# KMASAHIRO/AVR

Hardware: AMD Instinct MI355X
Metric: ray-samples/sec/GPU (1024 rays×256 samp×512 freq) + IR render ms/pose (higher is better)
Workload: dtype f32; 1 GPU; c2_meshrir_1024x256x512; mode=pose, rays=1024, samples=256, T=1022, freq_bins=512, distinct_poses=16, parallelism=poses x1 (no data-path collective)

## Files before the change

### avr_amd/csrc/render_bwd.hip

```cpp
#include "common.h"

using namespace avr;

typedef float floatx4 __attribute__((ext_vector_type(4)));

namespace {

constexpr int kBwdThreads = 256;
constexpr int kFc = 32;

__global__ __launch_bounds__(kBwdThreads) void dft_phase_bwd_kernel(
    avr_render_params pp, const float2* __restrict__ gout, const float* __restrict__ pl,
    const float2* __restrict__ phase, const float2* __restrict__ twg, float* __restrict__ gz, int B,
    int S, int T) {
    extern __shared__ float2 tw[];
    __shared__ float Au[16][kFc + 1];
    __shared__ float Av[16][kFc + 1];
    const int F = T / 2 + 1;
    const int b = blockIdx.z;
    const int s0 = blockIdx.y * 16;
    const int wave = threadIdx.x >> 6, lane = threadIdx.x & 63;
    const int t = blockIdx.x * 64 + wave * 16 + (lane & 15);
    const int tm = (t < T) ? t : 0;
    const int kq = lane >> 4;
    const int fo = kq >> 1, comp = kq & 1;
    const int srow = threadIdx.x >> 4, scol = 2 * (threadIdx.x & 15);
    const int ss = min(s0 + srow, S - 1);
    float2 ph_raw[2], g_raw[2];
    auto issue = [&](int fc) {
#pragma unroll
        for (int q = 0; q < 2; ++q) {
            const int f = min(fc + scol + q, F - 1);
            g_raw[q] = gout[(int64_t)b * F + f];
            ph_raw[q] = phase[(int64_t)ss * F + f];
        }
    };
    auto commit = [&](int fc) {
#pragma unroll
        for (int q = 0; q < 2; ++q) {
            const bool ok = (s0 + srow) < S && (fc + scol + q) < F;
            const float2 g = g_raw[q], ph = ph_raw[q];
            Au[srow][scol + q] = ok ? g.x * ph.x + g.y * ph.y : 0.0f;
            Av[srow][scol + q] = ok ? -(g.x * ph.y - g.y * ph.x) : 0.0f;
        }
    };
    issue(0);
    stage_table<kBwdThreads>(tw, twg, T);
    floatx4 acc = {0.0f, 0.0f, 0.0f, 0.0f};
    const int inc = (int)((2LL * tm) % T);
    for (int fc = 0; fc < F; fc += kFc) {
        __syncthreads();
        commit(fc);
        __syncthreads();
        if (fc + kFc < F) issue(fc + kFc);
        int idx = (int)(((int64_t)(fc + fo) * tm) % T);
#pragma unroll 4
        for (int ff = 0; ff < kFc; ff += 2) {
            const int r = lane & 15;
            const float a = comp ? Av[r][ff + fo] : Au[r][ff + fo];
            const float2 c = tw[idx];
            const float bv = comp ? c.y : c.x;
            acc = __builtin_amdgcn_mfma_f32_16x16x4f32(a, bv, acc, 0, 0, 0);
            idx += inc;
            if (idx >= T) idx -= T;
        }
    }
    float g4[4];
    int sh4[4];
#pragma unroll
    for (int reg = 0; reg < 4; ++reg) {
        const int s = min(s0 + 4 * kq + reg, S - 1);
        sh4[reg] = receiver_shift(pp, s);
        g4[reg] = pl[sh4[reg] + min(tm, T - 1)];
    }
    if (t < T) {
#pragma unroll
        for (int reg = 0; reg < 4; ++reg) {
            const int s = s0 + 4 * kq + reg;
            if (s < S) {
                const float v = (t < T - 1 - sh4[reg]) ? acc[reg] * g4[reg] : 0.0f;
                gz[((int64_t)b * S + s) * T + t] = v;
            }
        }
    }
}

constexpr int kMaxRbThreads = 1024;
constexpr int kMaxRbRays = 4096;

template <typename Tin, bool VECTOR, int CPT, int G, int MAXT, bool NTS>
__global__ __launch_bounds__(MAXT) void ray_reduce_bwd_kernel(
    avr_render_params pp, const Tin* __restrict__ sig, const float* __restrict__ gz, const float* __restrict__ w,
    const int32_t* __restrict__ delay, Tin* __restrict__ gsig, float* __restrict__ gw, int B,
    int R, int S, int T, int rays_per_split, int64_t total) {
    constexpr int VEC = VECTOR ? Vec16<Tin>::N : 1;
    extern __shared__ float lds_rb[];
    const int nthreads = blockDim.x, lane = threadIdx.x & 63;
    const int split = blockIdx.x, s0 = blockIdx.y * G, b = blockIdx.z;
    const int gcount = min(G, S - s0);
    const int r0 = split * rays_per_split;
    const int nr = max(0, min(R, r0 + rays_per_split) - r0);
    const int stride_l = G * max(nr, 1);
    float* w_l = lds_rb;
    int* d_l = reinterpret_cast<int*>(lds_rb + stride_l);
    float* dot_l = lds_rb + 2 * stride_l;
    for (int i = threadIdx.x; i < G * nr; i += nthreads) {
        const int g = i / nr, rr = i - g * nr;
        dot_l[i] = 0.0f;
        if (g < gcount) {
            const int64_t idx = ((int64_t)b * R + r0 + rr) * S + s0 + g;
            w_l[i] = w[idx];
            d_l[i] = delay[idx];
        } else {
            w_l[i] = 0.0f;
            d_l[i] = 0x7fffffff;
        }
    }
    const int64_t row0 = (((int64_t)b * R + r0) * S + s0) * (int64_t)T;
    const int L = gcount * T;
    const int phase = (int)(row0 % VEC);
    const int nchunks = (L + phase + VEC - 1) / VEC;
    const int64_t row_stride = (int64_t)S * T;

    float gv[CPT][VEC];
    int tk[CPT][VEC];
    int tm[CPT][VEC];
    int gk[CPT][VEC];
    int tmax[CPT][G];
    int lim[G];
    bool full[CPT];
    const float* gzc = gz + ((int64_t)b * S + s0) * T;
#pragma unroll
    for (int g = 0; g < G; ++g) lim[g] = tail_limit(pp, min(s0 + g, S - 1));
#pragma unroll
    for (int c = 0; c < CPT; ++c) {
        const int j = threadIdx.x + c * nthreads;
        const int ebase = j * VEC - phase;
        full[c] = j < nchunks && ebase >= 0 && ebase + VEC <= L;
#pragma unroll
        for (int g = 0; g < G; ++g) tmax[c][g] = -1;
#pragma unroll
        for (int k = 0; k < VEC; ++k) {
            const int e = ebase + k;
            const bool ok = j < nchunks && e >= 0 && e < L;
            const int g = (G == 1) ? 0 : (ok ? e / T : 0);
            gk[c][k] = g;
            tk[c][k] = ok ? e - g * T : -1;
            gv[c][k] = ok ? gzc[e] : 0.0f;
            int l = lim[0];
#pragma unroll
            for (int q = 1; q < G; ++q)
                if (g == q) l = lim[q];
            tm[c][k] = (tk[c][k] >= 0 && tk[c][k] < l) ? tk[c][k] : -1;
#pragma unroll
            for (int q = 0; q < G; ++q)
                if (g == q) tmax[c][q] = max(tmax[c][q], tm[c][k]);
        }
    }
    __syncthreads();

    auto live = [&](int r, int c) {
        bool any = false;
#pragma unroll
        for (int g = 0; g < G; ++g) any |= tmax[c][g] >= d_l[g * nr + r];
        return any;
    };
    auto load_chunk = [&](int64_t rowbase, int c, bool need, float* x) {
        const int j = threadIdx.x + c * nthreads;
        if constexpr (VECTOR) {
            load16_masked(sig + rowbase, (uint32_t)nchunks * 16u,
                          need ? (uint32_t)j * 16u : kSkip, x);
        } else {
            const int64_t e0 = rowbase + j;
            x[0] = (need && j < nchunks && e0 < total) ? load_f(sig, e0) : 0.0f;
        }
    };
    auto finish = [&](int r, int64_t rowbase, float (*x)[VEC]) {
        float wg[G], dotg[G];
        int dg[G];
#pragma unroll
        for (int g = 0; g < G; ++g) {
            wg[g] = w_l[g * nr + r];
            dg[g] = d_l[g * nr + r];
            dotg[g] = 0.0f;
        }
#pragma unroll
        for (int c = 0; c < CPT; ++c) {
            float o[VEC];
#pragma unroll
            for (int k = 0; k < VEC; ++k) {
                float ws = wg[0];
                int ds = dg[0];
#pragma unroll
                for (int g = 1; g < G; ++g)
                    if (gk[c][k] == g) {
                        ws = wg[g];
                        ds = dg[g];
                    }
                const float gm = (tm[c][k] >= ds) ? gv[c][k] : 0.0f;
                o[k] = ws * gm;
                const float pd = gm * x[c][k];
#pragma unroll
                for (int g = 0; g < G; ++g)
                    if (gk[c][k] == g) dotg[g] += pd;
            }
            const int j = threadIdx.x + c * nthreads;
            const int64_t e0 = rowbase + (int64_t)j * VEC;
            if (VECTOR && full[c]) {
                if constexpr (VECTOR) {
                    if constexpr (NTS)
                        store16_nt(gsig + e0, o);
                    else
                        store16(gsig + e0, o);
                }
            } else {
#pragma unroll
                for (int k = 0; k < VEC; ++k)
                    if (tk[c][k] >= 0) store_f(gsig, e0 + k, o[k]);
            }
        }
#pragma unroll
        for (int g = 0; g < G; ++g) {
            float v = dotg[g];
#pragma unroll
            for (int off = 32; off > 0; off >>= 1) v += __shfl_xor(v, off, 64);
            if (lane == 0) atomicAdd(&dot_l[g * nr + r], v);
        }
    };

    constexpr int U = 4;
    int r = 0;
    for (; r + U <= nr; r += U) {
        float x[U][CPT][VEC];
        bool need[U][CPT];
#pragma unroll
        for (int u = 0; u < U; ++u)
#pragma unroll
            for (int c = 0; c < CPT; ++c) need[u][c] = live(r + u, c);
#pragma unroll
        for (int u = 0; u < U; ++u) {
            const int64_t bu = row0 + (int64_t)(r + u) * row_stride - phase;
#pragma unroll
            for (int c = 0; c < CPT; ++c) load_chunk(bu, c, need[u][c], x[u][c]);
        }
#pragma unroll
        for (int u = 0; u < U; ++u) finish(r + u, row0 + (int64_t)(r + u) * row_stride - phase, x[u]);
    }
    for (; r < nr; ++r) {
        float xa[CPT][VEC];
        const int64_t ba = row0 + (int64_t)r * row_stride - phase;
#pragma unroll
        for (int c = 0; c < CPT; ++c) load_chunk(ba, c, live(r, c), xa[c]);
        finish(r, ba, xa);
    }
    __syncthreads();
    for (int i = threadIdx.x; i < G * nr; i += nthreads) {
        const int g = i / nr, rr = i - g * nr;
        if (g < gcount) gw[((int64_t)b * R + r0 + rr) * S + s0 + g] = dot_l[i];
    }
}

template <typename Ta>
__global__ void weights_bwd_kernel(avr_render_params p, int B, const Ta* __restrict__ attn,
                                   const float* __restrict__ d_vals,
                                   const float* __restrict__ grad_w, Ta* __restrict__ grad_attn,
                                   int waves_per_block) {
    extern __shared__ float lds[];
    const int R = n_rays(p), S = p.n_samples;
    const int wave = threadIdx.x >> 6, lane = threadIdx.x & 63;
    const int64_t ray = (int64_t)blockIdx.x * waves_per_block + wave;
    const bool active = ray < (int64_t)B * R;
    float* alpha = lds + (int64_t)wave * 4 * S;
    float* gwl = alpha + S;
    float* ex = gwl + S;
    float* dist = ex + S;
    const int64_t base = ray * S;
    if (active) {
        for (int s = lane; s < S; s += 64) {
            const float a = load_f(attn, base + s);
            const float d = d_vals[s];
            const float gap = (s + 1 < S) ? d_vals[s + 1] - d : 1e10f;
            const float e = expf(-a * gap);
            alpha[s] = 1.0f - e;
            ex[s] = e;
            dist[s] = gap;
            gwl[s] = grad_w[base + s];
        }
    }
    __syncthreads();
    if (!active) return;
    const int per = (S + 63) / 64;
    const int s0 = min(S, lane * per), s1 = min(S, s0 + per);
    float run = 1.0f;
    for (int s = s0; s < s1; ++s) run = run * ((1.0f - alpha[s]) + 1e-6f);
    float incl = run;
#pragma unroll
    for (int off = 1; off < 64; off <<= 1) {
        const float v = __shfl_up(incl, off, 64);
        if (lane >= off) incl = incl * v;
    }
    float trans0 = __shfl_up(incl, 1, 64);
    if (lane == 0) trans0 = 1.0f;
    float ca = 0.0f, cm = 1.0f;
    for (int s = s1 - 1; s >= s0; --s) {
        const float a_s = gwl[s] * alpha[s];
        const float m_s = (1.0f - alpha[s]) + 1e-6f;
        ca = a_s + m_s * ca;
        cm = m_s * cm;
    }
    float qa = ca, qm = cm;
#pragma unroll
    for (int off = 1; off < 64; off <<= 1) {
        const float na = __shfl_down(qa, off, 64);
        const float nm = __shfl_down(qm, off, 64);
        if (lane + off < 64) {
            qa = qa + qm * na;
            qm = qm * nm;
        }
    }
    float q = __shfl_down(qa, 1, 64);
    if (lane == 63) q = 0.0f;
    for (int s = s1 - 1; s >= s0; --s) {
        const float u_s = q;
        q = gwl[s] * alpha[s] + ((1.0f - alpha[s]) + 1e-6f) * q;
        gwl[s] = gwl[s] - u_s;
    }
    float tr = trans0;
    for (int s = s0; s < s1; ++s) {
        const float galpha = tr * gwl[s];
        const float gatt = (galpha * ex[s]) * dist[s];
        store_f(grad_attn, base + s, gatt);
        tr = tr * ((1.0f - alpha[s]) + 1e-6f);
    }
}

}

extern "C" int avr_dft_phase_bwd(const avr_render_params* p, int32_t B, const float* grad_out,
                                 const float* pl_table, const int32_t* shift, const float* phase,
                                 const float* twiddle, float* gz, void* stream) {
    AVR_REQUIRE(p && B >= 1 && grad_out && pl_table && shift && phase && twiddle && gz,
                "avr_dft_phase_bwd: bad args");
    const int S = p->n_samples, T = p->T;
    AVR_REQUIRE(T >= 2 && T <= 16384, "avr_dft_phase_bwd: T out of range");
    const dim3 grid((T + 63) / 64, (S + 15) / 16, B);
    const size_t lds = (size_t)T * sizeof(float2);
    (void)shift;
    if (lds > 65536)
        (void)hipFuncSetAttribute((const void*)dft_phase_bwd_kernel,
                                  hipFuncAttributeMaxDynamicSharedMemorySize, (int)lds);
    hipLaunchKernelGGL(dft_phase_bwd_kernel, grid, dim3(kBwdThreads), lds, as_stream(stream), *p,
                       reinterpret_cast<const float2*>(grad_out), pl_table,
                       reinterpret_cast<const float2*>(phase),
                       reinterpret_cast<const float2*>(twiddle), gz, (int)B, S, T);
    return check_launch("avr_dft_phase_bwd");
}

namespace {
template <typename Tin, bool VECTOR>
int launch_rb(const avr_render_params* p, int B, const void* sig, const float* gz, const float* w,
              const int32_t* delay, void* gsig, float* gw, hipStream_t st) {
    constexpr int VEC = VECTOR ? Vec16<Tin>::N : 1;
    const int R = n_rays(*p), S = p->n_samples, T = p->T;
    int G = 1;
    const int max_chunks = (VEC == 8) ? 256 : 512;
    while (G < 4 && 2 * G * T <= max_chunks * VEC && 2 * G <= S) G *= 2;
    int max_phase = 0;
    for (int s0 = 0; s0 < S && s0 < VEC * G; s0 += G)
        max_phase = max(max_phase, (int)(((int64_t)s0 * T) % VEC));
    const int nch = (G * T + max_phase + VEC - 1) / VEC;
    int cpt = 1;
    while ((nch + cpt - 1) / cpt > kMaxRbThreads) ++cpt;
    const int threads = max(64, ((nch + cpt - 1) / cpt + 63) / 64 * 64);
    const int groups = (S + G - 1) / G;
    int n = 1;
    const int64_t wps = (int64_t)groups * B * (threads / 64);
    const int64_t waves_target = 262144;
    auto rps_of = [&](int k) { return (R + k - 1) / k; };
    while (n < 256 && (n * wps < waves_target || rps_of(n) * G > kMaxRbRays) && rps_of(2 * n) >= 4) n *= 2;
    const int rps = rps_of(n);
    if (rps * G > kMaxRbRays) return fail(AVR_E_CONFIG, "ray_reduce_bwd: too many rays per split");
    const int64_t total = (int64_t)B * R * S * T;
    const dim3 grid((R + rps - 1) / rps, groups, B);
    const size_t lds = (size_t)3 * G * max(rps, 1) * 4;
    const Tin* x = (const Tin*)sig;
    Tin* gx = (Tin*)gsig;
    const bool nts = true;
#define AVR_RB_L(C, GG, MT, NTS)                                                                   \
    hipLaunchKernelGGL((ray_reduce_bwd_kernel<Tin, VECTOR, C, GG, MT, NTS>), grid, dim3(threads),  \
                       lds, st, *p, x, gz, w, delay, gx, gw, B, R, S, T, rps, total)
#define AVR_RB(C, GG)                                                                              \
    if (cpt == C && G == GG) {                                                                     \
        if (threads <= 512) {                                                                      \
            if (nts)                                                                               \
                AVR_RB_L(C, GG, 512, true);                                                        \
            else                                                                                   \
                AVR_RB_L(C, GG, 512, false);                                                       \
        } else {                                                                                   \
            if (nts)                                                                               \
                AVR_RB_L(C, GG, 1024, true);                                                       \
            else                                                                                   \
                AVR_RB_L(C, GG, 1024, false);                                                      \
        }                                                                                          \
        return check_launch("avr_ray_reduce_bwd");                                                 \
    }
    AVR_RB(1, 1) AVR_RB(1, 2) AVR_RB(1, 4) AVR_RB(2, 1) AVR_RB(2, 2) AVR_RB(2, 4) AVR_RB(3, 1)
    AVR_RB(4, 1)
#undef AVR_RB_L
#undef AVR_RB
    return fail(AVR_E_CONFIG, "ray_reduce_bwd: T too long for this build");
}
}

extern "C" int avr_ray_reduce_bwd(const avr_render_params* p, int32_t B, const void* signal,
                                  int32_t sig_dtype, const float* gz, const float* w,
                                  const int32_t* delay, void* grad_signal, float* grad_w,
                                  void* stream) {
    AVR_REQUIRE(p && B >= 1 && signal && gz && w && delay && grad_signal && grad_w,
                "avr_ray_reduce_bwd: bad args");
    AVR_REQUIRE(p->T >= 2 && p->T <= 16384, "avr_ray_reduce_bwd: T out of range");
    const int64_t st = (int64_t)p->n_samples * p->T;
    const bool aligned = (reinterpret_cast<uintptr_t>(signal) % 16) == 0 &&
                         (reinterpret_cast<uintptr_t>(grad_signal) % 16) == 0;
    hipStream_t s = as_stream(stream);
    if (sig_dtype == AVR_DTYPE_F32) {
        if (aligned && st % 4 == 0)
            return launch_rb<float, true>(p, B, signal, gz, w, delay, grad_signal, grad_w, s);
        return launch_rb<float, false>(p, B, signal, gz, w, delay, grad_signal, grad_w, s);
    }
    if (sig_dtype == AVR_DTYPE_F16) {
        if (aligned && st % 8 == 0)
            return launch_rb<__half, true>(p, B, signal, gz, w, delay, grad_signal, grad_w, s);
        return launch_rb<__half, false>(p, B, signal, gz, w, delay, grad_signal, grad_w, s);
    }
    if (sig_dtype == AVR_DTYPE_BF16) {
        if (aligned && st % 8 == 0)
            return launch_rb<__hip_bfloat16, true>(p, B, signal, gz, w, delay, grad_signal, grad_w, s);
        return launch_rb<__hip_bfloat16, false>(p, B, signal, gz, w, delay, grad_signal, grad_w, s);
    }
    return fail(AVR_E_ARG, "avr_ray_reduce_bwd: unknown signal dtype");
}

extern "C" int avr_weights_bwd(const avr_render_params* p, int32_t B, const void* attn,
                               int32_t attn_dtype, const float* d_vals, const float* grad_w,
                               void* grad_attn, void* stream) {
    AVR_REQUIRE(p && B >= 1 && attn && d_vals && grad_w && grad_attn, "avr_weights_bwd: bad args");
    const int S = p->n_samples;
    AVR_REQUIRE(S >= 1 && S <= 8192, "avr_weights_bwd: n_samples out of range");
    const int wpb = (S <= 1024) ? 4 : 1;
    const int64_t rays = (int64_t)B * n_rays(*p);
    const dim3 grid((unsigned)((rays + wpb - 1) / wpb));
    const size_t lds = (size_t)wpb * 4 * S * sizeof(float);
    if (lds > 65536) {
        if (attn_dtype == AVR_DTYPE_F32)
            (void)hipFuncSetAttribute((const void*)weights_bwd_kernel<float>,
                                hipFuncAttributeMaxDynamicSharedMemorySize, (int)lds);
        else if (attn_dtype == AVR_DTYPE_F16)
            (void)hipFuncSetAttribute((const void*)weights_bwd_kernel<__half>,
                                hipFuncAttributeMaxDynamicSharedMemorySize, (int)lds);
        else
            (void)hipFuncSetAttribute((const void*)weights_bwd_kernel<__hip_bfloat16>,
                                hipFuncAttributeMaxDynamicSharedMemorySize, (int)lds);
    }
    if (attn_dtype == AVR_DTYPE_F32)
        hipLaunchKernelGGL(weights_bwd_kernel<float>, grid, dim3(64 * wpb), lds, as_stream(stream),
                           *p, (int)B, (const float*)attn, d_vals, grad_w, (float*)grad_attn, wpb);
    else if (attn_dtype == AVR_DTYPE_F16)
        hipLaunchKernelGGL(weights_bwd_kernel<__half>, grid, dim3(64 * wpb), lds,
                           as_stream(stream), *p, (int)B, (const __half*)attn, d_vals, grad_w,
                           (__half*)grad_attn, wpb);
    else if (attn_dtype == AVR_DTYPE_BF16)
        hipLaunchKernelGGL(weights_bwd_kernel<__hip_bfloat16>, grid, dim3(64 * wpb), lds,
                           as_stream(stream), *p, (int)B, (const __hip_bfloat16*)attn, d_vals, grad_w,
                           (__hip_bfloat16*)grad_attn, wpb);
    else
        return fail(AVR_E_ARG, "avr_weights_bwd: unknown attn dtype");
    return check_launch("avr_weights_bwd");
}
```

### avr_amd/csrc/render_fwd.hip

```cpp
#include "common.h"

#include <cstdlib>

using namespace avr;

typedef float floatx16 __attribute__((ext_vector_type(16)));

namespace {

constexpr double kTwoPi = 6.283185307179586476925286766559;

__global__ void tables_kernel(avr_render_params p, float* __restrict__ d_vals,
                              float* __restrict__ frac, int32_t* __restrict__ shift,
                              float* __restrict__ pl, float2* __restrict__ phase,
                              float2* __restrict__ tw) {
    const int S = p.n_samples, T = p.T, F = T / 2 + 1;
    const int64_t gid = (int64_t)blockIdx.x * blockDim.x + threadIdx.x;
    const int64_t stride = (int64_t)gridDim.x * blockDim.x;
    for (int64_t i = gid; i < S; i += stride) {
        const float d = linspace_at(0.0f, 1.0f, S, (int)i) * p.depth_scale + p.depth_offset;
        const float fr = (p.fs * d) / p.speed;
        d_vals[i] = d;
        frac[i] = fr;
        shift[i] = (int32_t)rintf(fr);
// ... 239 lines not shown
        for (int s = lane; s < S; s += 64) w_out[base + s] = alpha[s];
}

constexpr int kMaxReduceThreads = 1024;
constexpr int kMaxGroupRays = 4096;

template <typename Tin, bool VECTOR, int CPT, int kUnroll, int G, int MAXT>
__global__ __launch_bounds__(MAXT) void ray_reduce_fwd_kernel(
    avr_render_params pp, const Tin* __restrict__ sig, const float* __restrict__ w,
    const int32_t* __restrict__ delay, float* __restrict__ part, int B, int R, int S, int T,
    int rays_per_split, int64_t total) {
    constexpr int VEC = VECTOR ? Vec16<Tin>::N : 1;
    extern __shared__ float lds_wd[];
    const int nthreads = blockDim.x;
    const int split = blockIdx.x, s0 = blockIdx.y * G, b = blockIdx.z;
    const int gcount = min(G, S - s0);
    const int r0 = split * rays_per_split;
    const int nr = max(0, min(R, r0 + rays_per_split) - r0);
    float* w_l = lds_wd;
    int* d_l = reinterpret_cast<int*>(lds_wd + G * max(nr, 1));
    for (int i = threadIdx.x; i < G * nr; i += nthreads) {
        const int g = i / nr, rr = i - g * nr;
        if (g < gcount) {
            const int64_t idx = ((int64_t)b * R + r0 + rr) * S + s0 + g;
            w_l[i] = w[idx];
            d_l[i] = delay[idx];
        } else {
            w_l[i] = 0.0f;
            d_l[i] = 0x7fffffff;
        }
    }
    __syncthreads();
    const int64_t row0 = (((int64_t)b * R + r0) * S + s0) * (int64_t)T;
    const int L = gcount * T;
    const int phase = (int)(row0 % VEC);
    const int nchunks = (L + phase + VEC - 1) / VEC;
    const int64_t row_stride = (int64_t)S * T;

    float acc[CPT][VEC];
    int tk[CPT][VEC];
    int tm[CPT][VEC];
    int gk[CPT][VEC];
    int tmax[CPT][G];
    int lim[G];
#pragma unroll
    for (int g = 0; g < G; ++g) lim[g] = tail_limit(pp, min(s0 + g, S - 1));
#pragma unroll
    for (int c = 0; c < CPT; ++c) {
#pragma unroll
        for (int g = 0; g < G; ++g) tmax[c][g] = -1;
#pragma unroll
        for (int k = 0; k < VEC; ++k) {
            acc[c][k] = 0.0f;
            const int e = (threadIdx.x + c * nthreads) * VEC + k - phase;
            const bool ok = e >= 0 && e < L;
            const int g = (G == 1) ? 0 : (ok ? e / T : 0);
            gk[c][k] = g;
            tk[c][k] = ok ? e - g * T : -1;
            int l = lim[0];
#pragma unroll
            for (int q = 1; q < G; ++q)
                if (g == q) l = lim[q];
            tm[c][k] = (tk[c][k] >= 0 && tk[c][k] < l) ? tk[c][k] : -1;
#pragma unroll
            for (int q = 0; q < G; ++q)
                if (g == q) tmax[c][q] = max(tmax[c][q], tm[c][k]);
        }
    }

    auto live = [&](int r, int c) {
        bool any = false;
#pragma unroll
        for (int g = 0; g < G; ++g) any |= tmax[c][g] >= d_l[g * nr + r];
        return any;
    };
    auto load_chunk = [&](int64_t rowbase, int c, bool need, float* x) {
        const int j = threadIdx.x + c * nthreads;
        if constexpr (VECTOR) {
            load16_masked(sig + rowbase, (uint32_t)nchunks * 16u,
                          need ? (uint32_t)j * 16u : kSkip, x);
        } else {
            const int64_t e0 = rowbase + j;
            x[0] = (need && j < nchunks && e0 < total) ? load_f(sig, e0) : 0.0f;
        }
    };
    auto accumulate = [&](int r, float (*x)[VEC]) {
        float wg[G];
        int dg[G];
#pragma unroll
        for (int g = 0; g < G; ++g) {
            wg[g] = w_l[g * nr + r];
            dg[g] = d_l[g * nr + r];
        }
#pragma unroll
        for (int c = 0; c < CPT; ++c)
#pragma unroll
            for (int k = 0; k < VEC; ++k) {
                float ws = wg[0];
                int ds = dg[0];
#pragma unroll
                for (int g = 1; g < G; ++g)
                    if (gk[c][k] == g) {
                        ws = wg[g];
                        ds = dg[g];
                    }
                const float wm = (tm[c][k] >= ds) ? ws : 0.0f;
                acc[c][k] = fmaf(wm, x[c][k], acc[c][k]);
            }
    };

    int r = 0;
    for (; r + kUnroll <= nr; r += kUnroll) {
        float x[kUnroll][CPT][VEC];
        bool need[kUnroll][CPT];
#pragma unroll
        for (int u = 0; u < kUnroll; ++u)
#pragma unroll
            for (int c = 0; c < CPT; ++c) need[u][c] = live(r + u, c);
#pragma unroll
        for (int u = 0; u < kUnroll; ++u) {
            const int64_t rowbase = row0 + (int64_t)(r + u) * row_stride - phase;
#pragma unroll
            for (int c = 0; c < CPT; ++c) load_chunk(rowbase, c, need[u][c], x[u][c]);
        }
#pragma unroll
        for (int u = 0; u < kUnroll; ++u) accumulate(r + u, x[u]);
    }
    for (; r < nr; ++r) {
        const int64_t rowbase = row0 + (int64_t)r * row_stride - phase;
        float x[CPT][VEC];
#pragma unroll
        for (int c = 0; c < CPT; ++c) load_chunk(rowbase, c, live(r, c), x[c]);
        accumulate(r, x);
    }
#pragma unroll
    for (int c = 0; c < CPT; ++c)
#pragma unroll
        for (int k = 0; k < VEC; ++k) {
            const int t = tk[c][k];
            if (t >= 0) part[(((int64_t)split * B + b) * S + s0 + gk[c][k]) * T + t] = acc[c][k];
        }
}

constexpr int kDftThreads = 256;
constexpr int kKc = 64;

template <int NS>
__global__ __launch_bounds__(kDftThreads) void dft_phase_fwd_kernel(
    avr_render_params pp, const float* __restrict__ part, const float* __restrict__ pl,
    const int32_t* __restrict__ shift, const float2* __restrict__ phase,
    const float2* __restrict__ twg, float2* __restrict__ spart, int B, int S, int T, int KS,
    int kchunk, int xcd_order) {
    extern __shared__ float2 tw[];
    __shared__ float As[32][kKc + 1];
    const int F = T / 2 + 1;
    const int P = ((S + 31) / 32) * KS;
    (void)P;
    const int nfb = (F + 127) / 128, nst = (S + 31) / 32;
    const int per = KS * nfb;
    int stile, q;
    if (xcd_order) {
        const int L = blockIdx.x, xcd = L & 7;
        q = L >> 3;
        stile = (q / per) * 8 + xcd;
        if (stile >= nst) return;
    } else {
        stile = blockIdx.x / per;
        q = blockIdx.x;
    }
    const int ks = (q % per) / nfb, fblk = (q % per) % nfb;
    const int b = blockIdx.z;
    const int wave = threadIdx.x >> 6, lane = threadIdx.x & 63;
    const int fbase = fblk * 128 + wave * 32;
    const int f = fbase + (lane & 31);
    const int fm = (f < F) ? f : 0;
    const int half = lane >> 5;
    const int col = threadIdx.x & 63, row0 = threadIdx.x >> 6;
    int sh[8];
    bool srow[8];
#pragma unroll
    for (int i = 0; i < 8; ++i) {
        const int s = stile * 32 + row0 + 4 * i;
        srow[i] = s < S;
        sh[i] = receiver_shift(pp, min(s, S - 1));
    }
    (void)shift;
    const int64_t slab = (int64_t)B * S * T;
    const int s_first = min(stile * 32 + row0, S - 1);
    const int64_t rowbase0 = ((int64_t)b * S + s_first) * T;
    const int64_t max_row_off = ((int64_t)b * S + (S - 1)) * T;

    const int k0 = ks * kchunk;
    const int k1 = min(T, k0 + kchunk);
    floatx16 acc_re, acc_im;
#pragma unroll
    for (int i = 0; i < 16; ++i) {
        acc_re[i] = 0.0f;
        acc_im[i] = 0.0f;
    }
    const int inc = (int)((2LL * fm) % T);
    float raw[NS][8], g[8];
    auto issue = [&](int kc) {
        const int tc = min(kc + col, T - 1);
#pragma unroll
        for (int k = 0; k < NS; ++k)
#pragma unroll
            for (int i = 0; i < 8; ++i) {
                const int64_t ro = min(rowbase0 + (int64_t)(4 * i) * T, max_row_off);
                raw[k][i] = part[k * slab + ro + tc];
            }
#pragma unroll
        for (int i = 0; i < 8; ++i) g[i] = pl[sh[i] + tc];
    };
    auto commit = [&](int kc) {
        const int t = kc + col;
#pragma unroll
        for (int i = 0; i < 8; ++i) {
            float sum = raw[0][i];
#pragma unroll
            for (int k = 1; k < NS; ++k) sum += raw[k][i];
            const bool ok = srow[i] && t < k1 && t < T - 1 - sh[i];
            As[row0 + 4 * i][col] = ok ? sum * g[i] : 0.0f;
        }
    };
    if (k0 < k1) issue(k0);
    stage_table<kDftThreads>(tw, twg, T);
    for (int kc = k0; kc < k1; kc += kKc) {
        __syncthreads();
        commit(kc);
        __syncthreads();
        if (kc + kKc < k1) issue(kc + kKc);
        int idx = (int)(((int64_t)(kc + half) * fm) % T);
#pragma unroll 8
        for (int kk = 0; kk < kKc; kk += 2) {
            const float a = As[lane & 31][kk + half];
            float2 c = tw[idx];
            asm volatile("" : "+v"(c.x), "+v"(c.y));
            acc_re = __builtin_amdgcn_mfma_f32_32x32x2f32(a, c.x, acc_re, 0, 0, 0);
            acc_im = __builtin_amdgcn_mfma_f32_32x32x2f32(a, c.y, acc_im, 0, 0, 0);
            idx += inc;
            if (idx >= T) idx -= T;
        }
    }
    float re = 0.0f, im = 0.0f;
    {
        float2 ph[16];
#pragma unroll
        for (int reg = 0; reg < 16; ++reg) {
            const int s = stile * 32 + (reg & 3) + 8 * (reg >> 2) + 4 * half;
            ph[reg] = phase[(int64_t)min(s, S - 1) * F + fm];
        }
#pragma unroll
        for (int reg = 0; reg < 16; ++reg) asm volatile("" ::"v"(ph[reg].x), "v"(ph[reg].y));
#pragma unroll
        for (int reg = 0; reg < 16; ++reg) {
            const int s = stile * 32 + (reg & 3) + 8 * (reg >> 2) + 4 * half;
            if (s < S) {
                const float zr = acc_re[reg], zi = acc_im[reg];
                re += zr * ph[reg].x - zi * ph[reg].y;
                im += zr * ph[reg].y + zi * ph[reg].x;
            }
        }
    }
    re += __shfl_xor(re, 32, 64);
    im += __shfl_xor(im, 32, 64);
    if (half == 0 && f < F) {
        spart[((int64_t)b * P + stile * KS + ks) * F + f] = make_float2(re, im);
    }
}

__global__ __launch_bounds__(256) void spectrum_finalize_kernel(int B, int P, int F,
                                                                const float2* __restrict__ spart,
                                                                float2* __restrict__ out) {
    __shared__ float2 red[16][17];
    const int b = blockIdx.y;
    const int g = threadIdx.x >> 4, j = threadIdx.x & 15;
    const int f = blockIdx.x * 16 + j;
    const int fc = min(f, F - 1);
    const float2* src = spart + (int64_t)b * P * F + fc;
    float ax = 0.f, ay = 0.f;
    for (int q0 = 0; q0 < P; q0 += 64) {
        float2 v[4];
#pragma unroll
        for (int u = 0; u < 4; ++u) v[u] = src[(int64_t)min(q0 + g + 16 * u, P - 1) * F];
#pragma unroll
        for (int u = 0; u < 4; ++u)
            if (q0 + g + 16 * u < P) {
                ax += v[u].x;
                ay += v[u].y;
            }
    }
    red[g][j] = make_float2(ax, ay);
    __syncthreads();
    if (g == 0 && f < F) {
        float2 r = red[0][j];
        for (int k = 1; k < 16; ++k) {
            r.x += red[k][j].x;
            r.y += red[k][j].y;
        }
        out[(int64_t)b * F + f] = r;
    }
}

__global__ __launch_bounds__(256) void irfft_kernel(int F, int B1, const float2* __restrict__ spec,
                                                    const float2* __restrict__ spec2,
                                                    const float2* __restrict__ twg,
                                                    float* __restrict__ ir, float* __restrict__ ir2) {
    extern __shared__ float2 lds[];
    __shared__ float red[8][33];
    const int n = 2 * (F - 1);
    float2* X = lds;
    float2* tw = lds + F;
    int b = blockIdx.y;
    if (b >= B1) {
        b -= B1;
        spec = spec2;
        ir = ir2;
    }
    stage_table<256>(X, spec + (int64_t)b * F, F);
    stage_table<256>(tw, twg, n);
    __syncthreads();
    const int tl = threadIdx.x & 31, slice = threadIdx.x >> 5;
    const int t = blockIdx.x * 32 + tl;
    const int tm = (t < n) ? t : 0;
    float acc[4] = {0.f, 0.f, 0.f, 0.f};
    int idx[4];
#pragma unroll
    for (int c = 0; c < 4; ++c) idx[c] = (int)(((int64_t)(1 + slice + 8 * c) * tm) % n);
    const int step4 = (int)((32LL * tm) % n);
    int k = 1 + slice;
    for (; k + 24 < F - 1; k += 32) {
#pragma unroll
        for (int c = 0; c < 4; ++c) {
            const float2 w = tw[idx[c]];
            const float2 x = X[k + 8 * c];
            acc[c] += x.x * w.x - x.y * w.y;
            idx[c] += step4;
            if (idx[c] >= n) idx[c] -= n;
        }
    }
    for (; k < F - 1; k += 8) {
        const int id = (int)(((int64_t)k * tm) % n);
        const float2 w = tw[id];
        const float2 x = X[k];
        acc[0] += x.x * w.x - x.y * w.y;
    }
    red[slice][tl] = (acc[0] + acc[1]) + (acc[2] + acc[3]);
    __syncthreads();
    if (slice == 0 && t < n) {
        float s = 0.0f;
#pragma unroll
        for (int q = 0; q < 8; ++q) s += red[q][tl];
        const float nyq = (t & 1) ? -X[F - 1].x : X[F - 1].x;
        const float v = (X[0].x + nyq) + 2.0f * s;
        ir[(int64_t)b * n + t] = v / (float)n;
    }
}

__global__ __launch_bounds__(256) void irfft_bwd_kernel(int F, const float* __restrict__ gir,
                                                        const float2* __restrict__ twg,
                                                        float2* __restrict__ grad) {
    extern __shared__ float lds_irb[];
    __shared__ float2 red[8][33];
    const int n = 2 * (F - 1);
    const int b = blockIdx.y;
    float2* tw = reinterpret_cast<float2*>(lds_irb);
    float* g = lds_irb + 2 * n;
    stage_table<256>(tw, twg, n);
    for (int i = threadIdx.x; i < n; i += 256) g[i] = gir[(int64_t)b * n + i];
    __syncthreads();
    const int kl = threadIdx.x & 31, sl = threadIdx.x >> 5;
    const int k = blockIdx.x * 32 + kl;
    const int km = k < F ? k : 0;
    int idx = (int)(((int64_t)km * sl) % n);
    const int step = (int)(((int64_t)km * 8) % n);
    float ac = 0.f, as = 0.f;
    for (int t = sl; t < n; t += 8) {
        const float2 c = tw[idx];
        ac = fmaf(g[t], c.x, ac);
        as = fmaf(g[t], c.y, as);
        idx += step;
        if (idx >= n) idx -= n;
    }
    red[sl][kl] = make_float2(ac, as);
    __syncthreads();
    if (sl == 0 && k < F) {
        float2 r = red[0][kl];
        for (int q = 1; q < 8; ++q) {
            r.x += red[q][kl].x;
            r.y += red[q][kl].y;
        }
        const bool edge = (k == 0) || (k == F - 1);
// ... 155 lines not shown
    }
    if (attn_dtype == AVR_DTYPE_F32)
        hipLaunchKernelGGL(weights_fwd_kernel<float>, grid, dim3(256), lds, as_stream(stream), *p,
                           (int)B, (const float*)attn, rays_o, pos_tx, dirs, d_vals, w, delay);
    else if (attn_dtype == AVR_DTYPE_F16)
        hipLaunchKernelGGL(weights_fwd_kernel<__half>, grid, dim3(256), lds, as_stream(stream),
                           *p, (int)B, (const __half*)attn, rays_o, pos_tx, dirs, d_vals, w, delay);
    else if (attn_dtype == AVR_DTYPE_BF16)
        hipLaunchKernelGGL(weights_fwd_kernel<__hip_bfloat16>, grid, dim3(256), lds,
                           as_stream(stream), *p, (int)B, (const __hip_bfloat16*)attn, rays_o,
                           pos_tx, dirs, d_vals, w, delay);
    else
        return fail(AVR_E_ARG, "avr_weights_fwd: unknown attn dtype");
    return check_launch("avr_weights_fwd");
}


namespace {
int reduce_variant() { return 2; }

struct ReduceShape {
    int G, cpt, threads;
};

template <int VEC>
ReduceShape reduce_shape(int S, int T) {
    ReduceShape sh;
    sh.G = 1;
    int max_phase = 0;
    for (int s0 = 0; s0 < S && s0 < VEC * sh.G; s0 += sh.G)
        max_phase = max(max_phase, (int)(((int64_t)s0 * T) % VEC));
    const int nch = (sh.G * T + max_phase + VEC - 1) / VEC;
    sh.cpt = 1;
    while ((nch + sh.cpt - 1) / sh.cpt > kMaxReduceThreads) ++sh.cpt;
    const int need = (nch + sh.cpt - 1) / sh.cpt;
    sh.threads = max(64, (need + 63) / 64 * 64);
    return sh;
}

template <typename Tin, bool VECTOR, int C, int G>
void launch_reduce_v(dim3 grid, dim3 block, size_t lds, hipStream_t st, const avr_render_params& pp,
                     const Tin* s, const float* w,
                     const int32_t* delay, float* part, int B, int R, int S, int T, int rps,
                     int64_t total) {
    const bool u8 = reduce_variant() == 3;
    if (block.x <= 512) {
        if (u8)
            hipLaunchKernelGGL((ray_reduce_fwd_kernel<Tin, VECTOR, C, 8, G, 512>), grid, block,
                               lds, st, pp, s, w, delay, part, B, R, S, T, rps, total);
        else
            hipLaunchKernelGGL((ray_reduce_fwd_kernel<Tin, VECTOR, C, 4, G, 512>), grid, block,
                               lds, st, pp, s, w, delay, part, B, R, S, T, rps, total);
    } else {
        if (u8)
            hipLaunchKernelGGL((ray_reduce_fwd_kernel<Tin, VECTOR, C, 8, G, 1024>), grid, block,
                               lds, st, pp, s, w, delay, part, B, R, S, T, rps, total);
        else
            hipLaunchKernelGGL((ray_reduce_fwd_kernel<Tin, VECTOR, C, 4, G, 1024>), grid, block,
                               lds, st, pp, s, w, delay, part, B, R, S, T, rps, total);
    }
}

template <typename Tin, bool VECTOR>
int launch_reduce(const avr_render_params* p, int B, const void* sig, const float* w,
                  const int32_t* delay, int n_split, float* part, hipStream_t st) {
    constexpr int VEC = VECTOR ? Vec16<Tin>::N : 1;
    const int R = n_rays(*p), S = p->n_samples, T = p->T;
    const int rps = (R + n_split - 1) / n_split;
    const ReduceShape sh = reduce_shape<VEC>(S, T);
    if (sh.G * rps > kMaxGroupRays)
        return fail(AVR_E_ARG, "avr_ray_reduce_fwd: too many rays per split (raise n_split)");
    const int64_t total = (int64_t)B * R * S * T;
    const dim3 grid(n_split, (S + sh.G - 1) / sh.G, B);
    const dim3 block(sh.threads);
    const size_t lds = (size_t)sh.G * max(rps, 1) * 8;
    const Tin* s = (const Tin*)sig;
#define AVR_RR(C, GG)                                                                              \
    if (sh.cpt == C && sh.G == GG)                                                                 \
        return launch_reduce_v<Tin, VECTOR, C, GG>(grid, block, lds, st, *p, s, w, delay, part, B, R, S, \
                                                   T, rps, total),                                 \
               check_launch("avr_ray_reduce_fwd");
    AVR_RR(1, 1) AVR_RR(1, 2) AVR_RR(1, 4) AVR_RR(2, 1) AVR_RR(2, 2) AVR_RR(2, 4) AVR_RR(3, 1)
    AVR_RR(4, 1)
#undef AVR_RR
    return fail(AVR_E_CONFIG, "ray_reduce: T too long for this build");
}
}

extern "C" int avr_reduce_splits(const avr_render_params* p, int32_t B, int32_t sig_dtype,
                                 int32_t* n_split) {
    if (int e = validate(p)) return e;
    AVR_REQUIRE(B >= 1 && n_split, "avr_reduce_splits: bad args");
    const int R = n_rays(*p), S = p->n_samples, T = p->T;
    const int vec = (sig_dtype == AVR_DTYPE_F16 || sig_dtype == AVR_DTYPE_BF16) ? 8 : 4;
    const ReduceShape sh = vec == 8 ? reduce_shape<8>(S, T) : reduce_shape<4>(S, T);
    const int groups = (S + sh.G - 1) / sh.G;
    auto rps = [&](int k) { return (R + k - 1) / k; };
    if (const char* f = getenv("AVR_NSPLIT")) {
        const int v = atoi(f);
        if ((v == 1 || v == 2 || v == 4 || v == 8 || v == 16) && v <= R && rps(v) * sh.G <= kMaxGroupRays) {
            *n_split = v;
            return 0;
        }
    }
    const int64_t waves_target = (vec == 8) ? 4096 : 1536;
    const int64_t waves_per_split = (int64_t)groups * B * (sh.threads / 64);
    int n = 1;
    while (n < 16 && (n * waves_per_split < waves_target || rps(n) * sh.G > kMaxGroupRays) &&
           rps(2 * n) >= 8)
        n *= 2;
    if (rps(n) * sh.G > kMaxGroupRays) return fail(AVR_E_CONFIG, "avr_reduce_splits: too many rays");
    *n_split = n;
    return 0;
}

extern "C" int avr_ray_reduce_fwd(const avr_render_params* p, int32_t B, const void* signal,
                                  int32_t sig_dtype, const float* w, const int32_t* delay,
                                  int32_t n_split, float* part, void* stream) {
    if (int e = validate(p)) return e;
    AVR_REQUIRE(B >= 1 && signal && w && delay && part, "avr_ray_reduce_fwd: null pointer");
    const int R = n_rays(*p);
    AVR_REQUIRE(n_split >= 1 && n_split <= R, "avr_ray_reduce_fwd: n_split out of range");
    AVR_REQUIRE((R + n_split - 1) / n_split <= kMaxGroupRays,
                "avr_ray_reduce_fwd: too many rays per split (raise n_split)");
    const int64_t st = (int64_t)p->n_samples * p->T;
    const bool aligned = (reinterpret_cast<uintptr_t>(signal) % 16) == 0;
    hipStream_t s = as_stream(stream);
    if (sig_dtype == AVR_DTYPE_F32) {
        if (aligned && st % 4 == 0) return launch_reduce<float, true>(p, B, signal, w, delay, n_split, part, s);
        return launch_reduce<float, false>(p, B, signal, w, delay, n_split, part, s);
    }
    if (sig_dtype == AVR_DTYPE_F16) {
        if (aligned && st % 8 == 0) return launch_reduce<__half, true>(p, B, signal, w, delay, n_split, part, s);
        return launch_reduce<__half, false>(p, B, signal, w, delay, n_split, part, s);
    }
    if (sig_dtype == AVR_DTYPE_BF16) {
        if (aligned && st % 8 == 0)
            return launch_reduce<__hip_bfloat16, true>(p, B, signal, w, delay, n_split, part, s);
        return launch_reduce<__hip_bfloat16, false>(p, B, signal, w, delay, n_split, part, s);
    }
    return fail(AVR_E_ARG, "avr_ray_reduce_fwd: unknown signal dtype");
}

extern "C" int avr_dft_phase_fwd(const avr_render_params* p, int32_t B, const float* part,
                                 int32_t n_split, const float* pl_table, const int32_t* shift,
                                 const float* phase, const float* twiddle, int32_t k_split,
                                 float* spart, void* stream) {
    if (int e = validate(p)) return e;
    AVR_REQUIRE(B >= 1 && part && pl_table && shift && phase && twiddle && spart,
                "avr_dft_phase_fwd: null pointer");
    const int S = p->n_samples, T = p->T, F = T / 2 + 1;
    const int nkc = (T + kKc - 1) / kKc;
    AVR_REQUIRE(k_split >= 1 && k_split <= nkc, "avr_dft_phase_fwd: k_split out of range");
    const int kchunk = ((nkc + k_split - 1) / k_split) * kKc;
    const int nst = (S + 31) / 32;
    const int xcd_order = nst >= 8;
    const int per = k_split * ((F + 127) / 128);
    const dim3 grid((unsigned)(xcd_order ? 8 * ((nst + 7) / 8) * per : nst * per), 1, B);
    const size_t lds = (size_t)T * sizeof(float2);
    auto go = [&](auto kern) {
        if (lds > 65536)
            (void)hipFuncSetAttribute((const void*)kern, hipFuncAttributeMaxDynamicSharedMemorySize,
                                      (int)lds);
        hipLaunchKernelGGL(kern, grid, dim3(kDftThreads), lds, as_stream(stream), *p, part, pl_table,
                           shift, reinterpret_cast<const float2*>(phase),
                           reinterpret_cast<const float2*>(twiddle),
                           reinterpret_cast<float2*>(spart), (int)B, S, T, (int)k_split, kchunk, xcd_order);
    };
    switch (n_split) {
        case 1: go(dft_phase_fwd_kernel<1>); break;
        case 2: go(dft_phase_fwd_kernel<2>); break;
        case 4: go(dft_phase_fwd_kernel<4>); break;
        case 8: go(dft_phase_fwd_kernel<8>); break;
        case 16: go(dft_phase_fwd_kernel<16>); break;
        default: return fail(AVR_E_ARG, "avr_dft_phase_fwd: n_split must be 1, 2, 4, 8 or 16");
    }
    return check_launch("avr_dft_phase_fwd");
}

extern "C" int avr_spectrum_finalize(int32_t B, int32_t P, int32_t F, const float* spart,
                                     float* out, void* stream) {
    AVR_REQUIRE(B >= 1 && P >= 1 && F >= 1 && spart && out, "avr_spectrum_finalize: bad args");
    hipLaunchKernelGGL(spectrum_finalize_kernel, dim3((unsigned)((F + 15) / 16), B), dim3(256), 0,
                       as_stream(stream), (int)B, (int)P, (int)F,
                       reinterpret_cast<const float2*>(spart), reinterpret_cast<float2*>(out));
    return check_launch("avr_spectrum_finalize");
}

namespace avr {
int launch_irfft(int B, int F, const float* spec, const float* spec2, const float* tw, float* ir,
                 float* ir2, void* stream) {
    AVR_REQUIRE(B >= 1 && F >= 2 && spec && tw && ir, "avr_irfft: bad args");
    const int n = 2 * (F - 1);
    AVR_REQUIRE(n <= 16384, "avr_irfft: n too large");
    const size_t lds = (size_t)(F + n) * sizeof(float2);
    const int rows = spec2 ? 2 * B : B;
    hipLaunchKernelGGL(irfft_kernel, dim3((n + 31) / 32, rows), dim3(256), lds, as_stream(stream),
                       (int)F, (int)B, reinterpret_cast<const float2*>(spec),
                       reinterpret_cast<const float2*>(spec2 ? spec2 : spec),
                       reinterpret_cast<const float2*>(tw), ir, ir2 ? ir2 : ir);
    return check_launch("avr_irfft");
}
}

extern "C" int avr_irfft(int32_t B, int32_t F, const float* spec, const float* tw, float* ir,
                         void* stream) {
    return avr::launch_irfft(B, F, spec, nullptr, tw, ir, nullptr, stream);
}

extern "C" int avr_irfft_bwd(int32_t B, int32_t F, const float* grad_ir, const float* tw,
                             float* grad_spec, void* stream) {
    AVR_REQUIRE(B >= 1 && F >= 2 && grad_ir && tw && grad_spec, "avr_irfft_bwd: bad args");
    const int n = 2 * (F - 1);
    const size_t lds = (size_t)n * (sizeof(float2) + sizeof(float));
    AVR_REQUIRE(lds <= 160 * 1024, "avr_irfft_bwd: n too large for LDS");
    if (lds > 65536)
        (void)hipFuncSetAttribute((const void*)irfft_bwd_kernel, hipFuncAttributeMaxDynamicSharedMemorySize,
                                  (int)lds);
    hipLaunchKernelGGL(irfft_bwd_kernel, dim3((F + 31) / 32, B), dim3(256), lds, as_stream(stream), (int)F,
                       grad_ir, reinterpret_cast<const float2*>(tw), reinterpret_cast<float2*>(grad_spec));
    return check_launch("avr_irfft_bwd");
}

namespace {
struct CoreLayout {
    int64_t w, delay, part, spart, bytes;
    int32_t n_split, k_split, P;
};

CoreLayout core_layout(const avr_render_params* p, int B, int sig_dtype) {
    CoreLayout L{};
    const int64_t R = n_rays(*p), S = p->n_samples, T = p->T, F = T / 2 + 1;
    int32_t ns = 1;
    avr_reduce_splits(p, B, sig_dtype, &ns);
    L.n_split = ns;
    const int nkc = (int)((T + kKc - 1) / kKc);
    int ks = 1;
    if (const char* f = getenv("AVR_KSPLIT")) {
        ks = atoi(f);
    } else {
        const int64_t base = ((F + 127) / 128) * ((S + 31) / 32) * B;
        ks = (int)((256 + (base > 0 ? base : 1) - 1) / (base > 0 ? base : 1));
    }
    if (ks < 1) ks = 1;
    if (ks > nkc) ks = nkc;
    L.k_split = ks;
    L.P = (int32_t)(((S + 31) / 32) * ks);
    auto al = [](int64_t x) { return (x + 255) & ~(int64_t)255; };
    int64_t o = 0;
    L.w = o;
    o += al((int64_t)B * R * S * 4);
    L.delay = o;
    o += al((int64_t)B * R * S * 4);
    L.part = o;
    o += al((int64_t)ns * B * S * T * 4);
    L.spart = o;
    o += al((int64_t)B * L.P * F * 8);
    L.bytes = o;
    return L;
}
}

extern "C" int avr_render_core_layout(const avr_render_params* p, int32_t B, int32_t sig_dtype,
                                      int64_t* offsets ,
                                      int32_t* splits ) {
    if (int e = validate(p)) return e;
    AVR_REQUIRE(B >= 1 && offsets && splits, "avr_render_core_layout: bad args");
    const CoreLayout L = core_layout(p, B, sig_dtype);
    offsets[0] = L.w;
    offsets[1] = L.delay;
    offsets[2] = L.part;
    offsets[3] = L.spart;
    offsets[4] = L.bytes;
    splits[0] = L.n_split;
    splits[1] = L.k_split;
    return 0;
}

extern "C" int avr_render_core_fwd(const avr_render_params* p, int32_t B, const void* attn,
                                   int32_t attn_dtype, const void* signal, int32_t sig_dtype,
                                   const float* rays_o, const float* pos_tx, const float* dirs,
                                   const avr_table_ptrs* tab, void* workspace,
                                   int64_t workspace_bytes, float* out, float* ir, void* ev_begin,
                                   void* ev_end, void* stream) {
    if (int e = validate(p)) return e;
    AVR_REQUIRE(tab && workspace && out, "avr_render_core_fwd: null pointer");
    const CoreLayout L = core_layout(p, B, sig_dtype);
    AVR_REQUIRE(workspace_bytes >= L.bytes, "avr_render_core_fwd: workspace too small");
    char* ws = reinterpret_cast<char*>(workspace);
    float* w = reinterpret_cast<float*>(ws + L.w);
    int32_t* delay = reinterpret_cast<int32_t*>(ws + L.delay);
    float* part = reinterpret_cast<float*>(ws + L.part);
    float* spart = reinterpret_cast<float*>(ws + L.spart);
    if (int e = avr_weights_fwd(p, B, attn, attn_dtype, rays_o, pos_tx, dirs, tab->d_vals, w, delay, stream))
        return e;
    hipStream_t s = as_stream(stream);
    if (ev_begin) (void)hipEventRecord(reinterpret_cast<hipEvent_t>(ev_begin), s);
    if (int e = avr_ray_reduce_fwd(p, B, signal, sig_dtype, w, delay, L.n_split, part, stream))
        return e;
    if (ev_end) (void)hipEventRecord(reinterpret_cast<hipEvent_t>(ev_end), s);
    if (int e = avr_dft_phase_fwd(p, B, part, L.n_split, tab->pl_table, tab->shift, tab->phase, tab->twiddle,
                                  L.k_split, spart, stream))
        return e;
    if (int e = avr_spectrum_finalize(B, L.P, p->T / 2 + 1, spart, out, stream)) return e;
    if (ir) {
        AVR_REQUIRE(tab->ir_twiddle, "avr_render_core_fwd: ir requested without ir_twiddle");
        return avr_irfft(B, p->T / 2 + 1, out, tab->ir_twiddle, ir, stream);
// ... 4 lines not shown
```

Before: 2.295 billion ray-samples/s.

## Exploit cos/sin symmetry to halve DFT work in forward and backward phase kernels

Both DFT kernels now fold time index t and T−t together, since cos is even and sin is odd. Forward uses summed and differenced inputs (Ae/Ao) over only the first half of the time range. Backward computes separate cosine and sine accumulators over half the outputs and writes both u and T−u. This roughly halves the MFMA and twiddle work, at the cost of extra gathers for the mirrored samples, a larger frequency chunk (kFc 128) with double-buffered register groups, and more complex boundary handling.

Result: no change. 2.311 billion ray-samples/s, median of 6 (+0.7%).

```diff
diff --git a/avr_amd/csrc/render_bwd.hip b/avr_amd/csrc/render_bwd.hip
--- a/avr_amd/csrc/render_bwd.hip
+++ b/avr_amd/csrc/render_bwd.hip
@@ -7,79 +7,113 @@
 namespace {
 
 constexpr int kBwdThreads = 256;
-constexpr int kFc = 32;
+constexpr int kFc = 128;
+constexpr int kFcPad = kFc + 2;
+constexpr int kStageQ = kFc / 16;
 
 __global__ __launch_bounds__(kBwdThreads) void dft_phase_bwd_kernel(
     avr_render_params pp, const float2* __restrict__ gout, const float* __restrict__ pl,
     const float2* __restrict__ phase, const float2* __restrict__ twg, float* __restrict__ gz, int B,
     int S, int T) {
     extern __shared__ float2 tw[];
-    __shared__ float Au[16][kFc + 1];
-    __shared__ float Av[16][kFc + 1];
-    const int F = T / 2 + 1;
+    __shared__ float Au[16][kFcPad];
+    __shared__ float Av[16][kFcPad];
+    const int F = T / 2 + 1, H = T / 2;
     const int b = blockIdx.z;
     const int s0 = blockIdx.y * 16;
     const int wave = threadIdx.x >> 6, lane = threadIdx.x & 63;
-    const int t = blockIdx.x * 64 + wave * 16 + (lane & 15);
-    const int tm = (t < T) ? t : 0;
+    const int u = blockIdx.x * 64 + wave * 16 + (lane & 15);
+    const int um = (u <= H) ? u : 0;
     const int kq = lane >> 4;
-    const int fo = kq >> 1, comp = kq & 1;
-    const int srow = threadIdx.x >> 4, scol = 2 * (threadIdx.x & 15);
+    const int srow = threadIdx.x >> 4, scol = threadIdx.x & 15;
     const int ss = min(s0 + srow, S - 1);
-    float2 ph_raw[2], g_raw[2];
+    float2 ph_raw[kStageQ], g_raw[kStageQ];
     auto issue = [&](int fc) {
 #pragma unroll
-        for (int q = 0; q < 2; ++q) {
-            const int f = min(fc + scol + q, F - 1);
+        for (int q = 0; q < kStageQ; ++q) {
+            const int f = min(fc + scol + 16 * q, F - 1);
             g_raw[q] = gout[(int64_t)b * F + f];
             ph_raw[q] = phase[(int64_t)ss * F + f];
         }
     };
     auto commit = [&](int fc) {
 #pragma unroll
-        for (int q = 0; q < 2; ++q) {
-            const bool ok = (s0 + srow) < S && (fc + scol + q) < F;
+        for (int q = 0; q < kStageQ; ++q) {
+            const bool ok = (s0 + srow) < S && (fc + scol + 16 * q) < F;
             const float2 g = g_raw[q], ph = ph_raw[q];
-            Au[srow][scol + q] = ok ? g.x * ph.x + g.y * ph.y : 0.0f;
-            Av[srow][scol + q] = ok ? -(g.x * ph.y - g.y * ph.x) : 0.0f;
+            Au[srow][scol + 16 * q] = ok ? g.x * ph.x + g.y * ph.y : 0.0f;
+            Av[srow][scol + 16 * q] = ok ? -(g.x * ph.y - g.y * ph.x) : 0.0f;
         }
     };
     issue(0);
     stage_table<kBwdThreads>(tw, twg, T);
-    floatx4 acc = {0.0f, 0.0f, 0.0f, 0.0f};
-    const int inc = (int)((2LL * tm) % T);
+    floatx4 acc_c = {0.0f, 0.0f, 0.0f, 0.0f};
+    floatx4 acc_s = {0.0f, 0.0f, 0.0f, 0.0f};
+    const int inc = (int)((4LL * um) % T);
     for (int fc = 0; fc < F; fc += kFc) {
         __syncthreads();
         commit(fc);
         __syncthreads();
         if (fc + kFc < F) issue(fc + kFc);
-        int idx = (int)(((int64_t)(fc + fo) * tm) % T);
-#pragma unroll 4
-        for (int ff = 0; ff < kFc; ff += 2) {
+        int idx = (int)(((int64_t)(fc + kq) * um) % T);
+        const int fend = min(kFc, (F - fc + 31) & ~31);
+        struct Group {
+            float au[4], av[4];
+            float2 c[4];
+        };
+        auto load = [&](int f0, Group& gq) {
             const int r = lane & 15;
-            const float a = comp ? Av[r][ff + fo] : Au[r][ff + fo];
-            const float2 c = tw[idx];
-            const float bv = comp ? c.y : c.x;
-            acc = __builtin_amdgcn_mfma_f32_16x16x4f32(a, bv, acc, 0, 0, 0);
-            idx += inc;
-            if (idx >= T) idx -= T;
-        }
-    }
-    float g4[4];
+#pragma unroll
+            for (int j = 0; j < 4; ++j) {
+                gq.au[j] = Au[r][f0 + 4 * j + kq];
+                gq.av[j] = Av[r][f0 + 4 * j + kq];
+                gq.c[j] = tw[idx];
+                idx += inc;
+                if (idx >= T) idx -= T;
+            }
+        };
+        auto run = [&](Group& gq) {
+#pragma unroll
+            for (int j = 0; j < 4; ++j) {
+                acc_c = __builtin_amdgcn_mfma_f32_16x16x4f32(gq.au[j], gq.c[j].x, acc_c, 0, 0, 0);
+                acc_s = __builtin_amdgcn_mfma_f32_16x16x4f32(gq.av[j], gq.c[j].y, acc_s, 0, 0, 0);
+            }
+            mfma_queue_wait();
+#pragma unroll
+            for (int j = 0; j < 4; ++j) {
+                keep_live(gq.c[j].x);
+                keep_live(gq.c[j].y);
+            }
+        };
+        Group ga, gb;
+        load(0, ga);
+        for (int f0 = 0; f0 < fend; f0 += 32) {
+            load(f0 + 16, gb);
+            run(ga);
+            load(min(f0 + 32, kFc - 16), ga);
+            run(gb);
+        }
+    }
+    const int tmr = min(T - um, T - 1);
+    const bool has_m = u >= 1 && 2 * u < T;
+    float g4[4], gm4[4];
     int sh4[4];
 #pragma unroll
     for (int reg = 0; reg < 4; ++reg) {
         const int s = min(s0 + 4 * kq + reg, S - 1);
         sh4[reg] = receiver_shift(pp, s);
-        g4[reg] = pl[sh4[reg] + min(tm, T - 1)];
-    }
-    if (t < T) {
+        g4[reg] = pl[sh4[reg] + um];
+        gm4[reg] = pl[sh4[reg] + tmr];
+    }
+    if (u <= H) {
 #pragma unroll
         for (int reg = 0; reg < 4; ++reg) {
             const int s = s0 + 4 * kq + reg;
             if (s < S) {
-                const float v = (t < T - 1 - sh4[reg]) ? acc[reg] * g4[reg] : 0.0f;
-                gz[((int64_t)b * S + s) * T + t] = v;
+                const int lim = T - 1 - sh4[reg];
+                float* row = gz + ((int64_t)b * S + s) * T;
+                row[u] = (u < lim) ? (acc_c[reg] + acc_s[reg]) * g4[reg] : 0.0f;
+                if (has_m) row[T - u] = (T - u < lim) ? (acc_c[reg] - acc_s[reg]) * gm4[reg] : 0.0f;
             }
         }
     }
@@ -343,7 +377,7 @@
                 "avr_dft_phase_bwd: bad args");
     const int S = p->n_samples, T = p->T;
     AVR_REQUIRE(T >= 2 && T <= 16384, "avr_dft_phase_bwd: T out of range");
-    const dim3 grid((T + 63) / 64, (S + 15) / 16, B);
+    const dim3 grid((T / 2 + 1 + 63) / 64, (S + 15) / 16, B);
     const size_t lds = (size_t)T * sizeof(float2);
     (void)shift;
     if (lds > 65536)
diff --git a/avr_amd/csrc/render_fwd.hip b/avr_amd/csrc/render_fwd.hip
--- a/avr_amd/csrc/render_fwd.hip
+++ b/avr_amd/csrc/render_fwd.hip
@@ -415,8 +415,9 @@
     const float2* __restrict__ twg, float2* __restrict__ spart, int B, int S, int T, int KS,
     int kchunk, int xcd_order) {
     extern __shared__ float2 tw[];
-    __shared__ float As[32][kKc + 1];
-    const int F = T / 2 + 1;
+    __shared__ float Ae[32][kKc + 1];
+    __shared__ float Ao[32][kKc + 1];
+    const int F = T / 2 + 1, H = T / 2;
     const int P = ((S + 31) / 32) * KS;
     (void)P;
     const int nfb = (F + 127) / 128, nst = (S + 31) / 32;
@@ -454,7 +455,7 @@
     const int64_t max_row_off = ((int64_t)b * S + (S - 1)) * T;
 
     const int k0 = ks * kchunk;
-    const int k1 = min(T, k0 + kchunk);
+    const int k1 = min(H + 1, k0 + kchunk);
     floatx16 acc_re, acc_im;
 #pragma unroll
     for (int i = 0; i < 16; ++i) {
@@ -462,28 +463,43 @@
         acc_im[i] = 0.0f;
     }
     const int inc = (int)((2LL * fm) % T);
-    float raw[NS][8], g[8];
+    float raw[NS][8], rawm[NS][8], g[8], gm[8];
     auto issue = [&](int kc) {
-        const int tc = min(kc + col, T - 1);
+        const int u = kc + col;
+        const int tc = min(u, T - 1);
+        const int tmc = min(max(T - u, 0), T - 1);
 #pragma unroll
         for (int k = 0; k < NS; ++k)
 #pragma unroll
             for (int i = 0; i < 8; ++i) {
                 const int64_t ro = min(rowbase0 + (int64_t)(4 * i) * T, max_row_off);
                 raw[k][i] = part[k * slab + ro + tc];
+                rawm[k][i] = part[k * slab + ro + tmc];
             }
 #pragma unroll
-        for (int i = 0; i < 8; ++i) g[i] = pl[sh[i] + tc];
+        for (int i = 0; i < 8; ++i) {
+            g[i] = pl[sh[i] + tc];
+            gm[i] = pl[sh[i] + tmc];
+        }
     };
     auto commit = [&](int kc) {
-        const int t = kc + col;
+        const int u = kc + col;
+        const bool has_m = u >= 1 && 2 * u < T;
 #pragma unroll
         for (int i = 0; i < 8; ++i) {
-            float sum = raw[0][i];
-#pragma unroll
-            for (int k = 1; k < NS; ++k) sum += raw[k][i];
-            const bool ok = srow[i] && t < k1 && t < T - 1 - sh[i];
-            As[row0 + 4 * i][col] = ok ? sum * g[i] : 0.0f;
+            float sum = raw[0][i], summ = rawm[0][i];
+#pragma unroll
+            for (int k = 1; k < NS; ++k) {
+                sum += raw[k][i];
+                summ += rawm[k][i];
+            }
+            const bool in = srow[i] && u < k1;
+            const bool ok = in && u < T - 1 - sh[i];
+            const bool okm = in && has_m && T - u < T - 1 - sh[i];
+            const float yd = ok ? sum * g[i] : 0.0f;
+            const float ym = okm ? summ * gm[i] : 0.0f;
+            Ae[row0 + 4 * i][col] = yd + ym;
+            Ao[row0 + 4 * i][col] = yd - ym;
         }
     };
     if (k0 < k1) issue(k0);
@@ -496,11 +512,12 @@
         int idx = (int)(((int64_t)(kc + half) * fm) % T);
 #pragma unroll 8
         for (int kk = 0; kk < kKc; kk += 2) {
-            const float a = As[lane & 31][kk + half];
+            const float ae = Ae[lane & 31][kk + half];
+            const float ao = Ao[lane & 31][kk + half];
             float2 c = tw[idx];
             asm volatile("" : "+v"(c.x), "+v"(c.y));
-            acc_re = __builtin_amdgcn_mfma_f32_32x32x2f32(a, c.x, acc_re, 0, 0, 0);
-            acc_im = __builtin_amdgcn_mfma_f32_32x32x2f32(a, c.y, acc_im, 0, 0, 0);
+            acc_re = __builtin_amdgcn_mfma_f32_32x32x2f32(ae, c.x, acc_re, 0, 0, 0);
+            acc_im = __builtin_amdgcn_mfma_f32_32x32x2f32(ao, c.y, acc_im, 0, 0, 0);
             idx += inc;
             if (idx >= T) idx -= T;
         }
@@ -962,7 +979,8 @@
     const int S = p->n_samples, T = p->T, F = T / 2 + 1;
     const int nkc = (T + kKc - 1) / kKc;
     AVR_REQUIRE(k_split >= 1 && k_split <= nkc, "avr_dft_phase_fwd: k_split out of range");
-    const int kchunk = ((nkc + k_split - 1) / k_split) * kKc;
+    const int nft = (T / 2 + 1 + kKc - 1) / kKc;
+    const int kchunk = ((nft + k_split - 1) / k_split) * kKc;
     const int nst = (S + 31) / 32;
     const int xcd_order = nst >= 8;
     const int per = k_split * ((F + 127) / 128);
```
